# dmiruke/find_motion

Measured on NVIDIA B200. Metric: 1080p frames/sec (whole box), higher is better.
Workload: dtype u8+f64

## Files before the change

find_motion_b200/csrc/fm_common.cuh:

```cuda
#pragma once

#include <cuda.h>
#include <cuda_runtime.h>
#include <stdint.h>

#include <atomic>
#include <utility>

#include "../../include/fm_gpu.h"
#include "fm_device.cuh"

#define FM_MAX_K 1024
#define FM_TILE_PX 512
#define FM_TILE_WORDS 16
#define FM_TIMING_RING 16384
#define FM_MAX_DEVICES 64

struct StreamState {
    int has_bg;
    int counter;
    int decay;
    int cache_len;
};

// ... 18 lines not shown
    int *parent;
    int *area2;
    int *bbox;
};

struct fm_ctx {
    fm_config cfg;
    fm_info info;
    int S, Tmax, W, H, w, h, k, wpr;
    int N;
    int ntiles;
    int resize_mode;
    size_t frame_bytes;
    uint8_t *nv12_bgr;
    bool fused;
    bool wide_fused;
    bool umma;
    uint8_t *uband;
    uint8_t *uband_f;
    bool umma_direct;
    int umma_ra;
    uint8_t *gpad;
    int fx, fy;
    int maxc;
    int *coef;
    uint32_t *wtab;
    ResizeTab xtab, ytab;
    int *g4start, *g4n, *g4off;
    float4 *g4w;
    int g4max;
// ... 76 lines not shown
#define FM_LAUNCH_CHECK()                                                         \
    do {                                                                          \
        g_launches.fetch_add(1, std::memory_order_relaxed);                       \
        cudaError_t e_ = cudaGetLastError();                                      \
        if (e_ != cudaSuccess) {                                                  \
            fm_set_error("kernel launch failed: %s (%s:%d)", cudaGetErrorString(e_), \
                         __FILE__, __LINE__);                                     \
            return FM_ECUDA;                                                      \
        }                                                                         \
    } while (0)

inline uint32_t *fm_tflat(const fm_ctx *c) {
    return c->tflat + (size_t)c->slot * c->S * c->Tmax * c->ntiles * FM_TILE_WORDS;
}
inline int *fm_rawrange(const fm_ctx *c) { return c->rawrange + (size_t)c->slot * 6 * c->S * c->Tmax; }

template <typename... KArgs, typename... Args>
cudaError_t fm_launch_chained(void (*kernel)(KArgs...), dim3 grid, dim3 block, size_t smem, cudaStream_t st,
                              Args &&...args) {
    cudaLaunchAttribute at[1];
    at[0].id = cudaLaunchAttributeProgrammaticStreamSerialization;
    at[0].val.programmaticStreamSerializationAllowed = 1;
    cudaLaunchConfig_t cfg = {};
    cfg.gridDim = grid; cfg.blockDim = block; cfg.dynamicSmemBytes = smem; cfg.stream = st;
    cfg.attrs = at; cfg.numAttrs = 1;
    return cudaLaunchKernelEx(&cfg, kernel, std::forward<Args>(args)...);
}
__device__ __forceinline__ unsigned long long fm_globaltimer() {
    unsigned long long t;
    asm volatile("mov.u64 %0, %%globaltimer;" : "=l"(t));
// ... 15 lines not shown
int fm_frames_tmap(const fm_ctx *c, const uint8_t *frames, size_t sstride, size_t fstride, int T, int box_words, int box_rows,
                   CUtensorMap *out);

int fm_launch_frontend(fm_ctx *c, const uint8_t *frames, size_t sstride, size_t fstride, int T,
                       cudaStream_t st);
int fm_launch_temporal(fm_ctx *c, int T, cudaStream_t st);
int fm_launch_fused(fm_ctx *c, const uint8_t *frames, size_t sstride, size_t fstride, int T, cudaStream_t st);
int fm_ccl_configure(fm_ctx *c);
int fm_launch_morph_ccl(fm_ctx *c, int T, cudaStream_t st, fm_frame_stats *stats_out);
int fm_launch_masks(fm_ctx *c, int stream, int n_polys, const int *offs, const int *pts_scaled,
                    int npts, cudaStream_t st);
int fm_launch_bg_export(fm_ctx *c, int stream, double *dst_dev, cudaStream_t st);
int fm_launch_thresh_export(fm_ctx *c, int stream, int t, uint8_t *dst_dev, cudaStream_t st);
int fm_launch_mask_export(fm_ctx *c, int stream, uint8_t *dst_dev, cudaStream_t st);
bool fm_fused_supported(const fm_ctx *c);
size_t fm_wide_plane_bytes(const fm_ctx *c);
int fm_wide_init(fm_ctx *c, const int *taps);
bool fm_wide_fused_supported(const fm_ctx *c);
size_t fm_wide_bg_doubles(const fm_ctx *c);
int fm_launch_bg_export_wide(fm_ctx *c, int stream, double *dst_dev, cudaStream_t st);
int fm_launch_wide_blur(fm_ctx *c, const uint8_t *frames, size_t sstride, size_t fstride, int T, cudaStream_t st);
size_t fm_fused_bg_doubles(const fm_ctx *c);
int fm_launch_bg_export_fused(fm_ctx *c, int stream, double *dst_dev, cudaStream_t st);
int fm_launch_resize_bgr(int device, const uint8_t *src_dev, size_t sstride, size_t fstride, int S, int T, int W, int H,
                         int w, int h, int mode, int fx, int fy, const ResizeTab &xt, const ResizeTab &yt, const int *oidx,
                         uint8_t *dst_dev, size_t ostride, cudaStream_t st);
size_t fm_upscale_smem(int w);
int fm_launch_upscale(int device, const uint8_t *frames, size_t sstride, size_t fstride, int T, int F, int W, int H, int w,
                      int h, const int2 *xt, const int2 *yt, const int *nvalid, uint8_t *gray, uint8_t *bgr_out,
                      const int *oidx, size_t ostride, cudaStream_t st);
// ... 30 lines not shown
```

find_motion_b200/csrc/fm_host.cu:

```cuda
#include <ctype.h>
#include <math.h>
#include <stdarg.h>
#include <stdio.h>
#include <stdlib.h>
#include <string.h>

#include <algorithm>
#include <map>
#include <mutex>
#include <utility>
#include <vector>

#include <sched.h>
#include <unistd.h>

#include "fm_common.cuh"

std::atomic<unsigned long long> g_launches{0};
static thread_local char g_err[512] = "";

int fm_ensure_smem(const void *func, size_t bytes, int device) {
    static std::mutex mu;
    static std::map<std::pair<const void *, int>, size_t> done;
    std::lock_guard<std::mutex> lk(mu);
// ... 379 lines not shown
    FM_TRY(cudaMemset(c->errflag, 0, sizeof(int)));
    FM_TRY(cudaMemset(c->heavy, 0, F * sizeof(int)));
    int cap = c->w / 4 + 3;
    size_t per_frame = (size_t)c->h * cap * 28 + (size_t)c->h * 4 + 4;
    size_t budget = (size_t)8 << 30;
    int nb = (int)std::min<size_t>(F, std::max<size_t>(1, budget / per_frame));
    if ((rc = fm_ccl_alloc(&c->ccl, nb, c->h, cap))) return fail(rc);
    if ((rc = fm_ccl_configure(c))) return fail(rc);
    if ((cfg->flags & FM_FLAG_DEVICE_CLIPS) && (rc = fm_clips_alloc(c))) return fail(rc);
#ifdef FM_NV12_STAGED
    const bool nv12_staged = true;
#else
    const bool nv12_staged = !c->fused;
#endif
    if ((cfg->flags & FM_FLAG_NV12) && nv12_staged) ALLOC(c->nv12_bgr, F * c->W * c->H * 3);
    if (cfg->flags & FM_FLAG_OBJECT_PLANES) {
        const int ow = FM_OBJECT_WIDTH;
        c->obj_h = obj_h;
        if (ow < c->W) {
            const double sx = 1.0 / ((double)ow / W), sy = 1.0 / ((double)obj_h / H);
            const int isx = (int)nearbyint(sx), isy = (int)nearbyint(sy);
            if (fabs(sx - isx) < 2.220446049250313e-16 && fabs(sy - isy) < 2.220446049250313e-16) {
                c->obj_mode = 2; c->obj_fx = isx; c->obj_fy = isy;
            } else {
                c->obj_mode = 1;
                const HostTab xt = area_tab(c->W, ow), yt = area_tab(c->H, obj_h);
                if ((rc = upload_tab(&c->obj_xtab, xt)) || (rc = upload_tab(&c->obj_ytab, yt))) return fail(rc);
                if ((rc = fm_rows_plan_objects(c, xt.start.data(), xt.idx.data(), xt.wt.data(), yt.start.data(), yt.idx.data())))
                    return fail(rc);
            }
// ... 573 lines not shown
```

find_motion_b200/csrc/k_fused.cu:

```cuda
#include <cuda.h>

#include "fm_common.cuh"

#define FT_W 128
#ifndef FT_H
#define FT_H 32
#endif
#define FT_PX 16
#define FUSED_WARPS (FT_H / 4)
#define FG_WORDS 36
#define FG_ROWS (FT_H + 4)
#define FH_MB ((FG_ROWS + 15) / 16)
#define FH_ROWS (16 * FH_MB)
#ifndef FUSED_MIN_CTAS
#define FUSED_MIN_CTAS (1024 / (8 * FT_H))
#endif
#define FH_WORDS 68
#define FUSED_THREADS (8 * FT_H)
#define RAW_PITCH 432
#define RAW_BYTES (RAW_PITCH * FG_ROWS)
#define RAW_STAGE ((RAW_BYTES + 127) / 128 * 128)
#define NV_PITCH 160
#define NV_Y_BYTES (NV_PITCH * FG_ROWS)
#define NV_BYTES (NV_Y_BYTES + NV_PITCH * FG_ROWS / 2)

struct FusedParams {
    int T, w, h, wpr;
    const int *nvalid;
    int tilesX, tilesY;
    double *bg;
    const uint32_t *maskbits;
    uint32_t *tbits;
    size_t flatwords;
    const int *bg_in;
    int *bg_out;
    int *clear_ff;
    int *clear_zero;
    int n_ff, n_zero;
    unsigned long long *stamp;
    int b0, b1, b2, shift, rnd;
    int threshold;
    double alpha, beta;
    int qoff; uint32_t nthr2; double nC;
    uint8_t *gray_out, *blur_out;
    int *rawrange;
    uint4 bfr[32];
#ifdef FM_K1_PROF
    long long *prof;
#endif
};

enum { K1_WAIT, K1_GRAY, K1_BORDER, K1_HORIZ, K1_VERT, K1_TAIL, K1_NPROF };
#ifdef FM_K1_PROF
#define K1_PROF(slot)                                \
    do {                                             \
        if (tid == 0) {                              \
            const long long now_ = clock64();        \
            k1_prof[slot] += now_ - k1_prof_t;       \
            k1_prof_t = now_;                        \
        }                                            \
    } while (0)
#else
#define K1_PROF(slot) do {} while (0)
#endif

static void fused_bfr(FusedParams &p) {
    for (int lane = 0; lane < 32; lane++) {
// ... 76 lines not shown
            fm_temporal_px<SAFE, INIT>(sv, bg[idx], bits, p.threshold, p.qoff, p.nthr2, p.alpha, p.beta, p.nC);
        }
    }
    return __brev(bits) >> (32 - FT_PX);
}

__device__ __forceinline__ void rawrange_hit(const FusedParams &p, int s, int t, int y) {
    int *rr = p.rawrange + 2 * ((size_t)s * p.T + t);
    atomicMax(rr, min(y + 3, p.h - 1));
    atomicMax(rr + 1, p.h - 1 - y);
}

__device__ __forceinline__ void fused_exit(const FusedParams &p) {
    fm_stamp_end(p.stamp);
    fm_wait_predecessor();
    const int nthreads = gridDim.x * gridDim.y * gridDim.z * FUSED_THREADS;
    for (int i = ((blockIdx.z * gridDim.y + blockIdx.y) * gridDim.x + blockIdx.x) * FUSED_THREADS + threadIdx.x;
         i < p.n_ff + p.n_zero; i += nthreads) {
        if (i < p.n_ff) p.clear_ff[i] = -1;
        else p.clear_zero[i - p.n_ff] = 0;
    }
}

__device__ __forceinline__ uint32_t nv12_gray4(uint32_t y4, const FmChroma &c0, const FmChroma &c1) {
    return fm_nv12_gray(y4 & 0xFFu, c0) | (fm_nv12_gray((y4 >> 8) & 0xFFu, c0) << 8) |
           (fm_nv12_gray((y4 >> 16) & 0xFFu, c1) << 16) | (fm_nv12_gray(y4 >> 24, c1) << 24);
}

template <bool KEEP, bool SAFE, bool NV12>
__global__ void __launch_bounds__(FUSED_THREADS, FUSED_MIN_CTAS) k_fused(const __grid_constant__ CUtensorMap tmap, FusedParams p,
                                                                         const __grid_constant__ CUtensorMap tmap_uv) {
    extern __shared__ __align__(128) unsigned char fsm[];
    unsigned char *raw = fsm;
    uint32_t *sg = reinterpret_cast<uint32_t *>(fsm + 2 * RAW_STAGE);
    uint32_t *sh = sg + FH_ROWS * FG_WORDS;
    uint64_t *bars = reinterpret_cast<uint64_t *>(sh + FH_ROWS * FH_WORDS);
    const int tid = threadIdx.x, lane = tid & 31, warp = tid >> 5;
    const int s = blockIdx.z;
    const int tx = blockIdx.x, ty = blockIdx.y, tile = ty * p.tilesX + tx;
    const int x0 = tx * FT_W, y0 = ty * FT_H;
    const int w = p.w, h = p.h;
    const bool border = (x0 == 0) || (x0 + FT_W >= w) || (y0 == 0) || (y0 + FT_H >= h);
    fm_stamp_start(p.stamp);
    const bool has_bg = p.bg_in[s] != 0;
    const int Ts = min(p.T, __ldg(p.nvalid + s));
    if (tid == 0 && tx == 0 && ty == 0) p.bg_out[s] = has_bg || Ts > 0;
    if (Ts <= 0) {
        fused_exit(p);
        return;
    }

    const int trow = tid >> 3, xg = tid & 7;
    const int px = x0 + 8 * xg, py = y0 + trow;
    double2 *bgt = reinterpret_cast<double2 *>(p.bg) +
                   ((((size_t)s * p.tilesX * p.tilesY + tile) * FUSED_WARPS + warp) * (FT_PX / 2)) * 32 + lane;
    double bg[FT_PX];
    if (has_bg) {
#pragma unroll
        for (int i = 0; i < FT_PX / 2; i++) {
            double2 v = bgt[i * 32];
            bg[2 * i] = v.x;
            bg[2 * i + 1] = v.y;
        }
    }
    uint32_t M = 0;
    const bool okA = py < h && px < w, okB = py < h && px + 64 < w;
    const uint32_t vmask = (okA ? 1u : 0u) | (okB ? 2u : 0u);
    if (okA) M = (__ldg(p.maskbits + ((size_t)s * h + py) * p.wpr + (px >> 5)) >> (px & 31)) & 0xFFu;
    if (okB) M |= ((__ldg(p.maskbits + ((size_t)s * h + py) * p.wpr + ((px + 64) >> 5)) >> (px & 31)) & 0xFFu) << 8;
    const bool wmasked = __any_sync(0xffffffffu, M != 0);
    const int cx = (x0 * 3) / 4 - 4, cy = y0 - 2;
    if (tid == 0) {
        fm_mbar_init(&bars[0], 1);
        fm_mbar_init(&bars[1], 1);
        asm volatile("fence.mbarrier_init.release.cluster;" ::: "memory");
        asm volatile("fence.proxy.async.shared::cta;" ::: "memory");
    }
    __syncthreads();
    if (tid == 0) {
        if (NV12) {
            fm_mbar_expect_tx(&bars[0], NV_BYTES);
            fm_tma_load_4d(raw, &tmap, &bars[0], x0 / 4 - 4, y0 - 2, 0, s);
            fm_tma_load_4d(raw + NV_Y_BYTES, &tmap_uv, &bars[0], x0 / 4 - 4, y0 / 2 - 1, 0, s);
        } else {
            fm_mbar_expect_tx(&bars[0], RAW_BYTES);
            fm_tma_load_4d(raw, &tmap, &bars[0], cx, cy, 0, s);
        }
    }
    uint8_t *tb = reinterpret_cast<uint8_t *>(p.tbits + ((size_t)s * p.T) * p.flatwords + (size_t)py * p.wpr) + (px >> 3);
    uint32_t bfr[2][2];
    {
        const uint4 b = p.bfr[lane];
        bfr[0][0] = b.x; bfr[0][1] = b.y; bfr[1][0] = b.z; bfr[1][1] = b.w;
        asm volatile("" : "+r"(bfr[0][0]), "+r"(bfr[0][1]), "+r"(bfr[1][0]), "+r"(bfr[1][1]));
    }
    const int hwin = warp & 7;
    const uint32_t sg_lane = fm_smem_u32(sg) + ((lane & 7) + 8 * ((lane >> 3) & 1)) * (FG_WORDS * 4) + 16 * hwin + 16 * (lane >> 4);
    uint32_t *sh_lane = sh + (lane >> 2) * FH_WORDS + 8 * hwin + (lane & 3);
    const int rs_tid = 4 + 24 * tid;
    uint2 *const sgt = reinterpret_cast<uint2 *>(sg) + tid;
    const uint32_t bars_s = fm_smem_u32(bars);
    uint32_t hits = 0;
#ifdef FM_K1_PROF
    long long k1_prof[K1_NPROF] = {}, k1_prof_t = clock64();
#endif

    for (int t = 0; t < Ts; t++) {
        if (tid == 0 && t + 1 < Ts) {
            if (NV12) {
                unsigned char *dst = raw + ((t + 1) & 1) * RAW_STAGE;
                fm_mbar_expect_tx(&bars[(t + 1) & 1], NV_BYTES);
                fm_tma_load_4d(dst, &tmap, &bars[(t + 1) & 1], x0 / 4 - 4, y0 - 2, t + 1, s);
                fm_tma_load_4d(dst + NV_Y_BYTES, &tmap_uv, &bars[(t + 1) & 1], x0 / 4 - 4, y0 / 2 - 1, t + 1, s);
            } else {
                fm_mbar_expect_tx(&bars[(t + 1) & 1], RAW_BYTES);
                fm_tma_load_4d(raw + ((t + 1) & 1) * RAW_STAGE, &tmap, &bars[(t + 1) & 1], cx, cy, t + 1, s);
            }
        }
        fm_mbar_wait(bars_s + 8 * (t & 1), (t >> 1) & 1);
        K1_PROF(K1_WAIT);
        if (NV12) {
            constexpr int NU = (FG_ROWS / 2) * FG_WORDS, NFULL = NU / FUSED_THREADS;
            const unsigned char *st = raw + (t & 1) * RAW_STAGE;
#pragma unroll
            for (int i = 0; i <= NFULL; i++) {
                if (i < NFULL || tid < NU - NFULL * FUSED_THREADS) {
                    const int un = tid + i * FUSED_THREADS, k = un / FG_WORDS, u = un - k * FG_WORDS;
                    const unsigned char *yq = st + 2 * k * NV_PITCH + 12 + 4 * u;
                    const uint32_t l0 = *reinterpret_cast<const uint32_t *>(yq);
                    const uint32_t l1 = *reinterpret_cast<const uint32_t *>(yq + NV_PITCH);
                    const uint32_t cw = *reinterpret_cast<const uint32_t *>(st + NV_Y_BYTES + k * NV_PITCH + 12 + 4 * u);
                    const FmChroma c0 = fm_nv12_chroma(cw & 0xFFu, (cw >> 8) & 0xFFu);
                    const FmChroma c1 = fm_nv12_chroma((cw >> 16) & 0xFFu, cw >> 24);
                    sg[2 * k * FG_WORDS + u] = nv12_gray4(l0, c0, c1);
                    sg[(2 * k + 1) * FG_WORDS + u] = nv12_gray4(l1, c0, c1);
                }
            }
        } else {
            constexpr int NU = FG_ROWS * FG_WORDS / 2, NFULL = NU / FUSED_THREADS;
            const unsigned char *rs = raw + (t & 1) * RAW_STAGE + rs_tid;
#pragma unroll
            for (int i = 0; i <= NFULL; i++) {
                if (i < NFULL || tid < NU - NFULL * FUSED_THREADS) {
                    const unsigned char *q = rs + i * (24 * FUSED_THREADS);
                    const uint32_t a0 = *reinterpret_cast<const uint32_t *>(q), a5 = *reinterpret_cast<const uint32_t *>(q + 20);
                    const uint2 a12 = *reinterpret_cast<const uint2 *>(q + 4), a34 = *reinterpret_cast<const uint2 *>(q + 12);
                    const uint32_t g0 = fm_gray4(a0, a12.x, a12.y), g1 = fm_gray4(a34.x, a34.y, a5);
                    sgt[i * FUSED_THREADS] = make_uint2(g0, g1);
                }
            }
        }
        __syncthreads();
        K1_PROF(K1_GRAY);
        if (border) {
            unsigned char *sb = reinterpret_cast<unsigned char *>(sg);
            for (int ry = tid; ry < FG_ROWS; ry += FUSED_THREADS) {
                unsigned char *row = sb + ry * (FG_WORDS * 4) + 4;
                if (x0 == 0) { row[-1] = row[1]; row[-2] = row[2]; }
                if (x0 + FT_W >= w) { int e = w - x0; row[e] = row[e - 2]; row[e + 1] = row[e - 3]; }
            }
            __syncthreads();
            for (int i = tid; i < FG_WORDS; i += FUSED_THREADS) {
                if (y0 == 0) { sg[1 * FG_WORDS + i] = sg[3 * FG_WORDS + i]; sg[0 * FG_WORDS + i] = sg[4 * FG_WORDS + i]; }
                if (y0 + FT_H >= h) {
                    int e = h - y0 + 2;
                    sg[e * FG_WORDS + i] = sg[(e - 2) * FG_WORDS + i];
                    sg[(e + 1) * FG_WORDS + i] = sg[(e - 3) * FG_WORDS + i];
                }
            }
            __syncthreads();
        }
        K1_PROF(K1_BORDER);
        if (KEEP) {
            for (int u = tid; u < FT_H * (FT_W / 4); u += FUSED_THREADS) {
                int ry = u / (FT_W / 4), ux = u - ry * (FT_W / 4);
                int gy = y0 + ry, gx = x0 + 4 * ux;
                if (gy < h && gx < w)
                    *reinterpret_cast<uint32_t *>(p.gray_out + (((size_t)s * p.T + t) * h + gy) * w + gx) =
                        sg[(ry + 2) * FG_WORDS + ux + 1];
            }
        }
        {
            constexpr int MBS = FUSED_WARPS / 8;
            constexpr int NMB = (FH_MB + MBS - 1) / MBS;
            const int mb0 = warp >> 3;
            uint32_t a[NMB][4];
#pragma unroll
            for (int i = 0; i < NMB; i++)
                if (MBS == 1 || mb0 + i * MBS < FH_MB) fm_ldsm_x4(sg_lane + (mb0 + i * MBS) * (16 * FG_WORDS * 4), a[i]);
#pragma unroll
            for (int i = 0; i < NMB; i++) {
                if (MBS == 1 || mb0 + i * MBS < FH_MB) {
                    int d0[4], d1[4];
                    fm_imma0(d0, a[i][0], a[i][1], a[i][2], a[i][3], bfr[0][0], bfr[0][1], 0);
                    fm_imma0(d1, a[i][0], a[i][1], a[i][2], a[i][3], bfr[1][0], bfr[1][1], 0);
                    uint32_t *o = sh_lane + (mb0 + i * MBS) * (16 * FH_WORDS);
                    o[0] = __byte_perm(d0[0], d0[1], 0x5410);
                    o[4] = __byte_perm(d1[0], d1[1], 0x5410);
                    o[8 * FH_WORDS] = __byte_perm(d0[2], d0[3], 0x5410);
                    o[8 * FH_WORDS + 4] = __byte_perm(d1[2], d1[3], 0x5410);
                }
            }
        }
        __syncthreads();
        K1_PROF(K1_HORIZ);
        const uint32_t *sgw = sh + trow * FH_WORDS + 4 * xg;
        asm volatile("" : "+r"(M));
        uint8_t *bo = KEEP ? p.blur_out + (((size_t)s * p.T + t) * h + py) * w + px : nullptr;
        uint32_t bits;
        if (t == 0 && !has_bg) bits = fused_rows<KEEP, SAFE, true, true, false>(sgw, bg, M, p, bo, vmask);
        else if (wmasked) bits = p.shift == 8 ? fused_rows<KEEP, SAFE, false, true, true>(sgw, bg, M, p, bo, vmask)
                                              : fused_rows<KEEP, SAFE, false, true, false>(sgw, bg, M, p, bo, vmask);
        else if (p.shift == 8) bits = fused_rows<KEEP, SAFE, false, false, true>(sgw, bg, M, p, bo, vmask);
        else bits = fused_rows<KEEP, SAFE, false, false, false>(sgw, bg, M, p, bo, vmask);
        K1_PROF(K1_VERT);
        if (!okA) bits = 0;
        if (!okB) bits &= 0xFFu;
        if (okA) tb[0] = (uint8_t)bits;
        if (okB) tb[8] = (uint8_t)(bits >> 8);
        const bool any = __any_sync(0xffffffffu, bits != 0);
        if (Ts <= 32) hits |= (any ? 1u : 0u) << t;
        else if (any && lane == 0) rawrange_hit(p, s, t, y0 + 4 * warp);
        tb += 4 * p.flatwords;
        K1_PROF(K1_TAIL);
    }
#ifdef FM_K1_PROF
    if (tid == 0) {
        for (int i = 0; i < K1_NPROF; i++) atomicAdd((unsigned long long *)p.prof + i, (unsigned long long)k1_prof[i]);
        atomicAdd((unsigned long long *)p.prof + K1_NPROF, (unsigned long long)Ts);
    }
#endif
    if (Ts <= 32 && ((hits >> lane) & 1u)) rawrange_hit(p, s, lane, y0 + 4 * warp);
#pragma unroll
    for (int i = 0; i < FT_PX / 2; i++) bgt[i * 32] = make_double2(bg[2 * i], bg[2 * i + 1]);
    fused_exit(p);
}

__global__ void k_bg_export_fused(const double *__restrict__ bg, double *__restrict__ dst, int w, int h, int tilesX,
                                  int tilesY, int s) {
    int x = blockIdx.x * blockDim.x + threadIdx.x, y = blockIdx.y;
    if (x >= w) return;
    int tx = x / FT_W, ty = y / FT_H, tile = ty * tilesX + tx;
    int lx = x - tx * FT_W, ly = y - ty * FT_H;
    int tid = ly * 8 + ((lx & 63) >> 3);
    int warp = tid >> 5, lane = tid & 31;
    int idx = 8 * (lx >> 6) + (lx & 7);
    size_t base = ((((size_t)s * tilesX * tilesY + tile) * FUSED_WARPS + warp) * (FT_PX / 2)) * 32;
    dst[(size_t)y * w + x] = bg[(base + (size_t)(idx >> 1) * 32 + lane) * 2 + (idx & 1)];
}
// ... 11 lines not shown
#include <cstdio>
#include <cstring>

static long long *k1_prof_buffer() {
    static long long *buf = nullptr;
    if (!buf && cudaMallocManaged(&buf, (K1_NPROF + 1) * sizeof(long long)) == cudaSuccess)
        memset(buf, 0, (K1_NPROF + 1) * sizeof(long long));
    return buf;
}

extern "C" void fm_k1_prof_dump(void) {
    long long *b = k1_prof_buffer();
    if (!b) return;
    cudaDeviceSynchronize();
    const double n = b[K1_NPROF] ? (double)b[K1_NPROF] : 1.0;
    fprintf(stderr, "k1 phases (cycles per CTA-frame, thread 0, %lld CTA-frames): wait %.1f gray %.1f border %.1f "
            "horizontal %.1f vertical %.1f tail %.1f\n", b[K1_NPROF], b[K1_WAIT] / n, b[K1_GRAY] / n, b[K1_BORDER] / n,
            b[K1_HORIZ] / n, b[K1_VERT] / n, b[K1_TAIL] / n);
    memset(b, 0, (K1_NPROF + 1) * sizeof(long long));
}
#endif

#define FUSED_SMEM (2 * RAW_STAGE + FH_ROWS * FG_WORDS * 4 + FH_ROWS * FH_WORDS * 4 + 16)

static int nv12_plane_tmap(const fm_ctx *c, const uint8_t *plane, int rows, size_t sstride, size_t fstride, int T,
                           int box_rows, CUtensorMap *out) {
    PFN_encodeTiled enc = fm_tma_encoder();
    if (!enc) { fm_set_error("cuTensorMapEncodeTiled not available"); return FM_ECUDA; }
    const size_t dense = c->frame_bytes;
    cuuint64_t dims[4] = {(cuuint64_t)c->W / 4, (cuuint64_t)rows, (cuuint64_t)T, (cuuint64_t)c->S};
    cuuint64_t strides[3] = {(cuuint64_t)c->W, (cuuint64_t)(T > 1 ? fstride : dense),
                             (cuuint64_t)(c->S > 1 ? sstride : (T > 1 ? fstride * T : dense))};
    cuuint32_t box[4] = {NV_PITCH / 4, (cuuint32_t)box_rows, 1, 1};
    cuuint32_t estr[4] = {1, 1, 1, 1};
    CUresult r = enc(out, CU_TENSOR_MAP_DATA_TYPE_UINT32, 4, (void *)plane, dims, strides, box, estr, CU_TENSOR_MAP_INTERLEAVE_NONE,
                     CU_TENSOR_MAP_SWIZZLE_NONE, CU_TENSOR_MAP_L2_PROMOTION_L2_128B, CU_TENSOR_MAP_FLOAT_OOB_FILL_NONE);
    if (r != CUDA_SUCCESS) { fm_set_error("cuTensorMapEncodeTiled (NV12 plane) failed (%d)", (int)r); return FM_ECUDA; }
    return FM_OK;
}

int fm_launch_fused(fm_ctx *c, const uint8_t *frames, size_t sstride, size_t fstride, int T, cudaStream_t st) {
    CUtensorMap tmap, tmap_uv;
    const bool nv12 = c->nv12_bgr == nullptr && (c->cfg.flags & FM_FLAG_NV12);
    int rc;
    if (nv12) {
        if ((((uintptr_t)frames) | sstride | fstride) & 15) {
            fm_set_error("the fused NV12 front end needs 16-byte aligned frames and strides");
            return FM_EINVAL;
        }
        if ((rc = nv12_plane_tmap(c, frames, c->H, sstride, fstride, T, FG_ROWS, &tmap))) return rc;
        if ((rc = nv12_plane_tmap(c, frames + (size_t)c->W * c->H, c->H / 2, sstride, fstride, T, FG_ROWS / 2, &tmap_uv))) return rc;
    } else {
        if ((rc = fm_frames_tmap(c, frames, sstride, fstride, T, RAW_PITCH / 4, FG_ROWS, &tmap))) return rc;
        tmap_uv = tmap;
    }
    FusedParams p;
    p.T = T; p.nvalid = c->nvalid;
    p.w = c->w; p.h = c->h; p.wpr = c->wpr;
    p.tilesX = (c->w + FT_W - 1) / FT_W; p.tilesY = (c->h + FT_H - 1) / FT_H;
    p.bg = c->bg; p.maskbits = c->maskbits; p.tbits = fm_tflat(c);
    p.flatwords = (size_t)c->ntiles * FM_TILE_WORDS;
    p.bg_in = c->bg_valid + (size_t)c->slot * c->S;
    p.bg_out = c->bg_valid + (size_t)(c->slot ^ 1) * c->S;
    {
        const int Fmax = c->S * c->Tmax;
        p.clear_ff = c->rawrange + (c->slot ? 0 : 2 * Fmax);
        p.n_ff = 6 * Fmax;
        p.clear_zero = c->ncomp;
        p.n_zero = 2 * Fmax + 4;
    }
    int lg;
    if (c->k == 1) { p.b0 = 0; p.b1 = 0; p.b2 = 1; lg = 8; }
    else if (c->k == 3) { p.b0 = 0; p.b1 = 1; p.b2 = 2; lg = 6; }
    else { p.b0 = 1; p.b1 = 4; p.b2 = 6; lg = 4; }
    p.shift = 16 - 2 * lg;
    int r1 = p.shift ? (1 << (p.shift - 1)) : 0;
    p.rnd = r1 | (r1 << 16);
    p.threshold = c->cfg.threshold;
    p.alpha = c->cfg.avg; p.beta = 1.0 - p.alpha;
    p.qoff = (int)(0x4B400000u - (unsigned)p.threshold); p.nthr2 = ~(2u * (unsigned)p.threshold); p.nC = -(4503599627370496.0 * p.alpha);
    p.gray_out = c->gray; p.blur_out = c->blur;
    p.rawrange = fm_rawrange(c);
    p.stamp = c->stamp;
#ifdef FM_K1_PROF
    p.prof = k1_prof_buffer();
    if (!p.prof) return FM_ECUDA;
#endif
    const bool keep = (c->cfg.flags & FM_FLAG_KEEP_PLANES) != 0;
    const bool safe = p.alpha >= 0.0 && p.alpha <= 1.0 && p.threshold >= 0;
    fused_bfr(p);
    dim3 grid(p.tilesX, p.tilesY, c->S);
    typedef void (*FusedKernel)(const CUtensorMap, FusedParams, const CUtensorMap);
    const FusedKernel kerns[2][2][2] = {{{k_fused<false, false, false>, k_fused<false, false, true>},
                                         {k_fused<false, true, false>, k_fused<false, true, true>}},
                                        {{k_fused<true, false, false>, k_fused<true, false, true>},
                                         {k_fused<true, true, false>, k_fused<true, true, true>}}};
    const FusedKernel kern = kerns[keep][safe][nv12];
    if ((rc = fm_ensure_smem((const void *)kern, FUSED_SMEM, c->cfg.device))) return rc;
    if (c->nv12_bgr) kern<<<grid, FUSED_THREADS, FUSED_SMEM, st>>>(tmap, p, tmap_uv);
    else (void)fm_launch_chained(kern, grid, dim3(FUSED_THREADS), FUSED_SMEM, st, tmap, p, tmap_uv);
    FM_LAUNCH_CHECK();
    return FM_OK;
}

int fm_launch_bg_export_fused(fm_ctx *c, int stream, double *dst_dev, cudaStream_t st) {
    dim3 grid((c->w + 127) / 128, c->h);
    k_bg_export_fused<<<grid, 128, 0, st>>>(c->bg, dst_dev, c->w, c->h, (c->w + FT_W - 1) / FT_W,
                                            (c->h + FT_H - 1) / FT_H, stream);
    FM_LAUNCH_CHECK();
    return FM_OK;
}
```

Measured before the change: 376,900.

## Convert fused front-end kernel to persistent CTAs with atomic tile work queue

The fused gray/blur/background kernel is changed from one CTA per (tile, stream) into a persistent grid sized to the number of resident CTAs. Each CTA pulls tiles from a global atomic counter. The TMA load for the next tile's first frame is issued during the current tile's last frame, and L2 prefetches of the next frame and of the next tile's background block are added. Border handling is folded into the gray conversion through row reflection and byte permutes, replacing the separate border pass. The aim is to remove launch and tail imbalance and hide load latency across tile boundaries, at the cost of atomic contention, a per-slot queue counter that must be cleared, and more complex index logic.

```diff
diff --git a/find_motion_b200/csrc/fm_common.cuh b/find_motion_b200/csrc/fm_common.cuh
--- a/find_motion_b200/csrc/fm_common.cuh
+++ b/find_motion_b200/csrc/fm_common.cuh
@@ -56,6 +56,7 @@
     size_t frame_bytes;
     uint8_t *nv12_bgr;
     bool fused;
+    int fused_ctas;
     bool wide_fused;
     bool umma;
     uint8_t *uband;
@@ -162,6 +163,7 @@
     return c->tflat + (size_t)c->slot * c->S * c->Tmax * c->ntiles * FM_TILE_WORDS;
 }
 inline int *fm_rawrange(const fm_ctx *c) { return c->rawrange + (size_t)c->slot * 6 * c->S * c->Tmax; }
+inline int *fm_k1_queue(const fm_ctx *c) { return c->ncomp + 2 * (size_t)c->S * c->Tmax + 2; }
 
 template <typename... KArgs, typename... Args>
 cudaError_t fm_launch_chained(void (*kernel)(KArgs...), dim3 grid, dim3 block, size_t smem, cudaStream_t st,
@@ -207,6 +209,7 @@
 int fm_launch_thresh_export(fm_ctx *c, int stream, int t, uint8_t *dst_dev, cudaStream_t st);
 int fm_launch_mask_export(fm_ctx *c, int stream, uint8_t *dst_dev, cudaStream_t st);
 bool fm_fused_supported(const fm_ctx *c);
+int fm_fused_init(fm_ctx *c);
 size_t fm_wide_plane_bytes(const fm_ctx *c);
 int fm_wide_init(fm_ctx *c, const int *taps);
 bool fm_wide_fused_supported(const fm_ctx *c);
diff --git a/find_motion_b200/csrc/fm_host.cu b/find_motion_b200/csrc/fm_host.cu
--- a/find_motion_b200/csrc/fm_host.cu
+++ b/find_motion_b200/csrc/fm_host.cu
@@ -417,6 +417,7 @@
     const bool nv12_staged = !c->fused;
 #endif
     if ((cfg->flags & FM_FLAG_NV12) && nv12_staged) ALLOC(c->nv12_bgr, F * c->W * c->H * 3);
+    if (c->fused && (rc = fm_fused_init(c))) return fail(rc);
     if (cfg->flags & FM_FLAG_OBJECT_PLANES) {
         const int ow = FM_OBJECT_WIDTH;
         c->obj_h = obj_h;
diff --git a/find_motion_b200/csrc/k_fused.cu b/find_motion_b200/csrc/k_fused.cu
--- a/find_motion_b200/csrc/k_fused.cu
+++ b/find_motion_b200/csrc/k_fused.cu
@@ -1,4 +1,6 @@
 #include <cuda.h>
+
+#include <algorithm>
 
 #include "fm_common.cuh"
 
@@ -28,6 +30,9 @@
     int T, w, h, wpr;
     const int *nvalid;
     int tilesX, tilesY;
+    int tiles, items;
+    int *queue;
+    int *queue_clear;
     double *bg;
     const uint32_t *maskbits;
     uint32_t *tbits;
@@ -50,7 +55,7 @@
 #endif
 };
 
-enum { K1_WAIT, K1_GRAY, K1_BORDER, K1_HORIZ, K1_VERT, K1_TAIL, K1_NPROF };
+enum { K1_WAIT, K1_GRAY, K1_HORIZ, K1_VERT, K1_TAIL, K1_NPROF };
 #ifdef FM_K1_PROF
 #define K1_PROF(slot)                                \
     do {                                             \
@@ -157,11 +162,62 @@
 __device__ __forceinline__ void fused_exit(const FusedParams &p) {
     fm_stamp_end(p.stamp);
     fm_wait_predecessor();
-    const int nthreads = gridDim.x * gridDim.y * gridDim.z * FUSED_THREADS;
-    for (int i = ((blockIdx.z * gridDim.y + blockIdx.y) * gridDim.x + blockIdx.x) * FUSED_THREADS + threadIdx.x;
-         i < p.n_ff + p.n_zero; i += nthreads) {
+    const int nthreads = gridDim.x * FUSED_THREADS;
+    for (int i = blockIdx.x * FUSED_THREADS + threadIdx.x; i <= p.n_ff + p.n_zero; i += nthreads) {
         if (i < p.n_ff) p.clear_ff[i] = -1;
-        else p.clear_zero[i - p.n_ff] = 0;
+        else if (i < p.n_ff + p.n_zero) p.clear_zero[i - p.n_ff] = 0;
+        else *p.queue_clear = 0;
+    }
+}
+
+__device__ __forceinline__ int fused_src_row(int r, int y0, int h) {
+    if (y0 == 0 && r < 2) return 4 - r;
+    const int e = h - y0 + 2;
+    return (r == e || r == e + 1) ? 2 * e - 2 - r : r;
+}
+
+__device__ __forceinline__ void fused_item(const FusedParams &p, int it, int &s, int &tile, int &x0, int &y0) {
+    s = it / p.tiles;
+    tile = it - s * p.tiles;
+    const int ty = tile / p.tilesX;
+    x0 = (tile - ty * p.tilesX) * FT_W;
+    y0 = ty * FT_H;
+}
+
+__device__ __forceinline__ int fused_take(const FusedParams &p, int &ts) {
+    for (;;) {
+        const int it = atomicAdd(p.queue, 1);
+        if (it >= p.items) return p.items;
+        const int s = it / p.tiles;
+        ts = min(p.T, __ldg(p.nvalid + s));
+        if (it == s * p.tiles) p.bg_out[s] = p.bg_in[s] != 0 || ts > 0;
+        if (ts > 0) return it;
+    }
+}
+
+__device__ __forceinline__ void fm_tma_prefetch_4d(const CUtensorMap *map, int c0, int c1, int c2, int c3) {
+    asm volatile("cp.async.bulk.prefetch.tensor.4d.L2.global.tile [%0, {%1, %2, %3, %4}];"
+                 ::"l"(map), "r"(c0), "r"(c1), "r"(c2), "r"(c3) : "memory");
+}
+__device__ __forceinline__ void fm_bulk_prefetch(const void *src, uint32_t bytes) {
+    asm volatile("cp.async.bulk.prefetch.L2.global [%0], %1;" ::"l"(src), "r"(bytes) : "memory");
+}
+
+template <bool NV12>
+__device__ __forceinline__ void fused_load(unsigned char *dst, uint64_t *bar, const CUtensorMap *tmap, const CUtensorMap *tmap_uv,
+                                           int x0, int y0, int t, int s, bool next) {
+    if (NV12) {
+        fm_mbar_expect_tx(bar, NV_BYTES);
+        fm_tma_load_4d(dst, tmap, bar, x0 / 4 - 4, y0 - 2, t, s);
+        fm_tma_load_4d(dst + NV_Y_BYTES, tmap_uv, bar, x0 / 4 - 4, y0 / 2 - 1, t, s);
+        if (next) {
+            fm_tma_prefetch_4d(tmap, x0 / 4 - 4, y0 - 2, t + 1, s);
+            fm_tma_prefetch_4d(tmap_uv, x0 / 4 - 4, y0 / 2 - 1, t + 1, s);
+        }
+    } else {
+        fm_mbar_expect_tx(bar, RAW_BYTES);
+        fm_tma_load_4d(dst, tmap, bar, (x0 * 3) / 4 - 4, y0 - 2, t, s);
+        if (next) fm_tma_prefetch_4d(tmap, (x0 * 3) / 4 - 4, y0 - 2, t + 1, s);
     }
 }
 
@@ -178,59 +234,11 @@
     uint32_t *sg = reinterpret_cast<uint32_t *>(fsm + 2 * RAW_STAGE);
     uint32_t *sh = sg + FH_ROWS * FG_WORDS;
     uint64_t *bars = reinterpret_cast<uint64_t *>(sh + FH_ROWS * FH_WORDS);
+    __shared__ int next_item[2];
     const int tid = threadIdx.x, lane = tid & 31, warp = tid >> 5;
-    const int s = blockIdx.z;
-    const int tx = blockIdx.x, ty = blockIdx.y, tile = ty * p.tilesX + tx;
-    const int x0 = tx * FT_W, y0 = ty * FT_H;
     const int w = p.w, h = p.h;
-    const bool border = (x0 == 0) || (x0 + FT_W >= w) || (y0 == 0) || (y0 + FT_H >= h);
     fm_stamp_start(p.stamp);
-    const bool has_bg = p.bg_in[s] != 0;
-    const int Ts = min(p.T, __ldg(p.nvalid + s));
-    if (tid == 0 && tx == 0 && ty == 0) p.bg_out[s] = has_bg || Ts > 0;
-    if (Ts <= 0) {
-        fused_exit(p);
-        return;
-    }
-
     const int trow = tid >> 3, xg = tid & 7;
-    const int px = x0 + 8 * xg, py = y0 + trow;
-    double2 *bgt = reinterpret_cast<double2 *>(p.bg) +
-                   ((((size_t)s * p.tilesX * p.tilesY + tile) * FUSED_WARPS + warp) * (FT_PX / 2)) * 32 + lane;
-    double bg[FT_PX];
-    if (has_bg) {
-#pragma unroll
-        for (int i = 0; i < FT_PX / 2; i++) {
-            double2 v = bgt[i * 32];
-            bg[2 * i] = v.x;
-            bg[2 * i + 1] = v.y;
-        }
-    }
-    uint32_t M = 0;
-    const bool okA = py < h && px < w, okB = py < h && px + 64 < w;
-    const uint32_t vmask = (okA ? 1u : 0u) | (okB ? 2u : 0u);
-    if (okA) M = (__ldg(p.maskbits + ((size_t)s * h + py) * p.wpr + (px >> 5)) >> (px & 31)) & 0xFFu;
-    if (okB) M |= ((__ldg(p.maskbits + ((size_t)s * h + py) * p.wpr + ((px + 64) >> 5)) >> (px & 31)) & 0xFFu) << 8;
-    const bool wmasked = __any_sync(0xffffffffu, M != 0);
-    const int cx = (x0 * 3) / 4 - 4, cy = y0 - 2;
-    if (tid == 0) {
-        fm_mbar_init(&bars[0], 1);
-        fm_mbar_init(&bars[1], 1);
-        asm volatile("fence.mbarrier_init.release.cluster;" ::: "memory");
-        asm volatile("fence.proxy.async.shared::cta;" ::: "memory");
-    }
-    __syncthreads();
-    if (tid == 0) {
-        if (NV12) {
-            fm_mbar_expect_tx(&bars[0], NV_BYTES);
-            fm_tma_load_4d(raw, &tmap, &bars[0], x0 / 4 - 4, y0 - 2, 0, s);
-            fm_tma_load_4d(raw + NV_Y_BYTES, &tmap_uv, &bars[0], x0 / 4 - 4, y0 / 2 - 1, 0, s);
-        } else {
-            fm_mbar_expect_tx(&bars[0], RAW_BYTES);
-            fm_tma_load_4d(raw, &tmap, &bars[0], cx, cy, 0, s);
-        }
-    }
-    uint8_t *tb = reinterpret_cast<uint8_t *>(p.tbits + ((size_t)s * p.T) * p.flatwords + (size_t)py * p.wpr) + (px >> 3);
     uint32_t bfr[2][2];
     {
         const uint4 b = p.bfr[lane];
@@ -243,139 +251,210 @@
     const int rs_tid = 4 + 24 * tid;
     uint2 *const sgt = reinterpret_cast<uint2 *>(sg) + tid;
     const uint32_t bars_s = fm_smem_u32(bars);
-    uint32_t hits = 0;
+    if (tid == 0) {
+        fm_mbar_init(&bars[0], 1);
+        fm_mbar_init(&bars[1], 1);
+        asm volatile("fence.mbarrier_init.release.cluster;" ::: "memory");
+        asm volatile("fence.proxy.async.shared::cta;" ::: "memory");
+        int ts = 0;
+        const int it = fused_take(p, ts);
+        next_item[0] = it;
+        if (it < p.items) {
+            int s, tile, x0, y0;
+            fused_item(p, it, s, tile, x0, y0);
+            fused_load<NV12>(raw, &bars[0], &tmap, &tmap_uv, x0, y0, 0, s, ts > 1);
+        }
+    }
+    __syncthreads();
+    uint32_t f = 0;
 #ifdef FM_K1_PROF
     long long k1_prof[K1_NPROF] = {}, k1_prof_t = clock64();
 #endif
-
-    for (int t = 0; t < Ts; t++) {
-        if (tid == 0 && t + 1 < Ts) {
-            if (NV12) {
-                unsigned char *dst = raw + ((t + 1) & 1) * RAW_STAGE;
-                fm_mbar_expect_tx(&bars[(t + 1) & 1], NV_BYTES);
-                fm_tma_load_4d(dst, &tmap, &bars[(t + 1) & 1], x0 / 4 - 4, y0 - 2, t + 1, s);
-                fm_tma_load_4d(dst + NV_Y_BYTES, &tmap_uv, &bars[(t + 1) & 1], x0 / 4 - 4, y0 / 2 - 1, t + 1, s);
-            } else {
-                fm_mbar_expect_tx(&bars[(t + 1) & 1], RAW_BYTES);
-                fm_tma_load_4d(raw + ((t + 1) & 1) * RAW_STAGE, &tmap, &bars[(t + 1) & 1], cx, cy, t + 1, s);
+    for (int n = 0;; n++) {
+        const int it = next_item[n & 1];
+        if (it >= p.items) break;
+        int s, tile, x0, y0;
+        fused_item(p, it, s, tile, x0, y0);
+        const bool border = (x0 == 0) || (x0 + FT_W >= w) || (y0 == 0) || (y0 + FT_H + 1 >= h);
+        const bool has_bg = p.bg_in[s] != 0;
+        const int Ts = min(p.T, __ldg(p.nvalid + s));
+        const int px = x0 + 8 * xg, py = y0 + trow;
+        double2 *bgt = reinterpret_cast<double2 *>(p.bg) + (((size_t)it * FUSED_WARPS + warp) * (FT_PX / 2)) * 32 + lane;
+        double bg[FT_PX];
+        if (has_bg) {
+#pragma unroll
+            for (int i = 0; i < FT_PX / 2; i++) {
+                double2 v = bgt[i * 32];
+                bg[2 * i] = v.x;
+                bg[2 * i + 1] = v.y;
             }
         }
-        fm_mbar_wait(bars_s + 8 * (t & 1), (t >> 1) & 1);
-        K1_PROF(K1_WAIT);
-        if (NV12) {
-            constexpr int NU = (FG_ROWS / 2) * FG_WORDS, NFULL = NU / FUSED_THREADS;
-            const unsigned char *st = raw + (t & 1) * RAW_STAGE;
-#pragma unroll
-            for (int i = 0; i <= NFULL; i++) {
-                if (i < NFULL || tid < NU - NFULL * FUSED_THREADS) {
-                    const int un = tid + i * FUSED_THREADS, k = un / FG_WORDS, u = un - k * FG_WORDS;
-                    const unsigned char *yq = st + 2 * k * NV_PITCH + 12 + 4 * u;
-                    const uint32_t l0 = *reinterpret_cast<const uint32_t *>(yq);
-                    const uint32_t l1 = *reinterpret_cast<const uint32_t *>(yq + NV_PITCH);
-                    const uint32_t cw = *reinterpret_cast<const uint32_t *>(st + NV_Y_BYTES + k * NV_PITCH + 12 + 4 * u);
-                    const FmChroma c0 = fm_nv12_chroma(cw & 0xFFu, (cw >> 8) & 0xFFu);
-                    const FmChroma c1 = fm_nv12_chroma((cw >> 16) & 0xFFu, cw >> 24);
-                    sg[2 * k * FG_WORDS + u] = nv12_gray4(l0, c0, c1);
-                    sg[(2 * k + 1) * FG_WORDS + u] = nv12_gray4(l1, c0, c1);
+        uint32_t M = 0;
+        const bool okA = py < h && px < w, okB = py < h && px + 64 < w;
+        const uint32_t vmask = (okA ? 1u : 0u) | (okB ? 2u : 0u);
+        if (okA) M = (__ldg(p.maskbits + ((size_t)s * h + py) * p.wpr + (px >> 5)) >> (px & 31)) & 0xFFu;
+        if (okB) M |= ((__ldg(p.maskbits + ((size_t)s * h + py) * p.wpr + ((px + 64) >> 5)) >> (px & 31)) & 0xFFu) << 8;
+        const bool wmasked = __any_sync(0xffffffffu, M != 0);
+        uint8_t *tb = reinterpret_cast<uint8_t *>(p.tbits + ((size_t)s * p.T) * p.flatwords + (size_t)py * p.wpr) + (px >> 3);
+        uint32_t hits = 0;
+
+        for (int t = 0; t < Ts; t++, f++) {
+            if (tid == 0) {
+                unsigned char *dst = raw + ((f + 1) & 1) * RAW_STAGE;
+                uint64_t *bar = &bars[(f + 1) & 1];
+                if (t + 1 < Ts) {
+                    fused_load<NV12>(dst, bar, &tmap, &tmap_uv, x0, y0, t + 1, s, t + 2 < Ts);
+                } else {
+                    int ts = 0;
+                    const int nx = fused_take(p, ts);
+                    next_item[(n + 1) & 1] = nx;
+                    if (nx < p.items) {
+                        int ns, ntile, nx0, ny0;
+                        fused_item(p, nx, ns, ntile, nx0, ny0);
+                        fused_load<NV12>(dst, bar, &tmap, &tmap_uv, nx0, ny0, 0, ns, ts > 1);
+                        if (p.bg_in[ns] != 0)
+                            fm_bulk_prefetch(reinterpret_cast<const double2 *>(p.bg) + (size_t)nx * FUSED_WARPS * (FT_PX / 2) * 32,
+                                             FUSED_WARPS * (FT_PX / 2) * 32 * sizeof(double2));
+                    }
                 }
             }
-        } else {
-            constexpr int NU = FG_ROWS * FG_WORDS / 2, NFULL = NU / FUSED_THREADS;
-            const unsigned char *rs = raw + (t & 1) * RAW_STAGE + rs_tid;
-#pragma unroll
-            for (int i = 0; i <= NFULL; i++) {
-                if (i < NFULL || tid < NU - NFULL * FUSED_THREADS) {
-                    const unsigned char *q = rs + i * (24 * FUSED_THREADS);
-                    const uint32_t a0 = *reinterpret_cast<const uint32_t *>(q), a5 = *reinterpret_cast<const uint32_t *>(q + 20);
-                    const uint2 a12 = *reinterpret_cast<const uint2 *>(q + 4), a34 = *reinterpret_cast<const uint2 *>(q + 12);
-                    const uint32_t g0 = fm_gray4(a0, a12.x, a12.y), g1 = fm_gray4(a34.x, a34.y, a5);
-                    sgt[i * FUSED_THREADS] = make_uint2(g0, g1);
+            fm_mbar_wait(bars_s + 8 * (f & 1), (f >> 1) & 1);
+            K1_PROF(K1_WAIT);
+            if (NV12) {
+                constexpr int NU = (FG_ROWS / 2) * FG_WORDS, NFULL = NU / FUSED_THREADS;
+                const unsigned char *st = raw + (f & 1) * RAW_STAGE;
+#pragma unroll
+                for (int i = 0; i <= NFULL; i++) {
+                    if (i < NFULL || tid < NU - NFULL * FUSED_THREADS) {
+                        const int un = tid + i * FUSED_THREADS, k = un / FG_WORDS, u = un - k * FG_WORDS;
+                        if (!border) {
+                            const unsigned char *yq = st + 2 * k * NV_PITCH + 12 + 4 * u;
+                            const uint32_t l0 = *reinterpret_cast<const uint32_t *>(yq);
+                            const uint32_t l1 = *reinterpret_cast<const uint32_t *>(yq + NV_PITCH);
+                            const uint32_t cw = *reinterpret_cast<const uint32_t *>(st + NV_Y_BYTES + k * NV_PITCH + 12 + 4 * u);
+                            const FmChroma c0 = fm_nv12_chroma(cw & 0xFFu, (cw >> 8) & 0xFFu);
+                            const FmChroma c1 = fm_nv12_chroma((cw >> 16) & 0xFFu, cw >> 24);
+                            sg[2 * k * FG_WORDS + u] = nv12_gray4(l0, c0, c1);
+                            sg[(2 * k + 1) * FG_WORDS + u] = nv12_gray4(l1, c0, c1);
+                        } else {
+                            const int r0 = fused_src_row(2 * k, y0, h), r1 = fused_src_row(2 * k + 1, y0, h);
+                            int us = u;
+                            uint32_t sel = 0x3210;
+                            if (x0 == 0 && u == 0) { us = 1; sel = 0x1200; }
+                            if (x0 + FT_W >= w && u == (w - x0) / 4 + 1) { us = u - 1; sel = 0x3212; }
+                            const unsigned char *yq = st + 12 + 4 * us, *cq = st + NV_Y_BYTES + 12 + 4 * us;
+                            const uint32_t l0 = *reinterpret_cast<const uint32_t *>(yq + r0 * NV_PITCH);
+                            const uint32_t l1 = *reinterpret_cast<const uint32_t *>(yq + r1 * NV_PITCH);
+                            uint32_t cw = *reinterpret_cast<const uint32_t *>(cq + (r0 >> 1) * NV_PITCH);
+                            FmChroma c0 = fm_nv12_chroma(cw & 0xFFu, (cw >> 8) & 0xFFu);
+                            FmChroma c1 = fm_nv12_chroma((cw >> 16) & 0xFFu, cw >> 24);
+                            sg[2 * k * FG_WORDS + u] = __byte_perm(nv12_gray4(l0, c0, c1), 0, sel);
+                            if ((r1 >> 1) != (r0 >> 1)) {
+                                cw = *reinterpret_cast<const uint32_t *>(cq + (r1 >> 1) * NV_PITCH);
+                                c0 = fm_nv12_chroma(cw & 0xFFu, (cw >> 8) & 0xFFu);
+                                c1 = fm_nv12_chroma((cw >> 16) & 0xFFu, cw >> 24);
+                            }
+                            sg[(2 * k + 1) * FG_WORDS + u] = __byte_perm(nv12_gray4(l1, c0, c1), 0, sel);
+                        }
+                    }
                 }
-            }
-        }
-        __syncthreads();
-        K1_PROF(K1_GRAY);
-        if (border) {
-            unsigned char *sb = reinterpret_cast<unsigned char *>(sg);
-            for (int ry = tid; ry < FG_ROWS; ry += FUSED_THREADS) {
-                unsigned char *row = sb + ry * (FG_WORDS * 4) + 4;
-                if (x0 == 0) { row[-1] = row[1]; row[-2] = row[2]; }
-                if (x0 + FT_W >= w) { int e = w - x0; row[e] = row[e - 2]; row[e + 1] = row[e - 3]; }
-            }
-            __syncthreads();
-            for (int i = tid; i < FG_WORDS; i += FUSED_THREADS) {
-                if (y0 == 0) { sg[1 * FG_WORDS + i] = sg[3 * FG_WORDS + i]; sg[0 * FG_WORDS + i] = sg[4 * FG_WORDS + i]; }
-                if (y0 + FT_H >= h) {
-                    int e = h - y0 + 2;
-                    sg[e * FG_WORDS + i] = sg[(e - 2) * FG_WORDS + i];
-                    sg[(e + 1) * FG_WORDS + i] = sg[(e - 3) * FG_WORDS + i];
+            } else {
+                constexpr int NU = FG_ROWS * FG_WORDS / 2, NFULL = NU / FUSED_THREADS;
+                if (border) {
+                    const unsigned char *stg = raw + (f & 1) * RAW_STAGE + 4;
+                    const int ecu = x0 + FT_W >= w ? (w - x0) / 8 : -1;
+#pragma unroll
+                    for (int i = 0; i <= NFULL; i++) {
+                        if (i < NFULL || tid < NU - NFULL * FUSED_THREADS) {
+                            const int un = tid + i * FUSED_THREADS, r = un / (FG_WORDS / 2), c = un - r * (FG_WORDS / 2);
+                            const unsigned char *q = stg + fused_src_row(r, y0, h) * RAW_PITCH + 24 * c;
+                            const uint32_t a0 = *reinterpret_cast<const uint32_t *>(q), a5 = *reinterpret_cast<const uint32_t *>(q + 20);
+                            const uint2 a12 = *reinterpret_cast<const uint2 *>(q + 4), a34 = *reinterpret_cast<const uint2 *>(q + 12);
+                            uint32_t g0 = fm_gray4(a0, a12.x, a12.y), g1 = fm_gray4(a34.x, a34.y, a5);
+                            if (x0 == 0 && c == 0) g0 = __byte_perm(g0, g1, 0x5610);
+                            if (c == ecu) g1 = __byte_perm(g1, g0, 0x3256);
+                            sgt[i * FUSED_THREADS] = make_uint2(g0, g1);
+                        }
+                    }
+                } else {
+                    const unsigned char *rs = raw + (f & 1) * RAW_STAGE + rs_tid;
+#pragma unroll
+                    for (int i = 0; i <= NFULL; i++) {
+                        if (i < NFULL || tid < NU - NFULL * FUSED_THREADS) {
+                            const unsigned char *q = rs + i * (24 * FUSED_THREADS);
+                            const uint32_t a0 = *reinterpret_cast<const uint32_t *>(q), a5 = *reinterpret_cast<const uint32_t *>(q + 20);
+                            const uint2 a12 = *reinterpret_cast<const uint2 *>(q + 4), a34 = *reinterpret_cast<const uint2 *>(q + 12);
+                            const uint32_t g0 = fm_gray4(a0, a12.x, a12.y), g1 = fm_gray4(a34.x, a34.y, a5);
+                            sgt[i * FUSED_THREADS] = make_uint2(g0, g1);
+                        }
+                    }
                 }
             }
             __syncthreads();
-        }
-        K1_PROF(K1_BORDER);
-        if (KEEP) {
-            for (int u = tid; u < FT_H * (FT_W / 4); u += FUSED_THREADS) {
-                int ry = u / (FT_W / 4), ux = u - ry * (FT_W / 4);
-                int gy = y0 + ry, gx = x0 + 4 * ux;
-                if (gy < h && gx < w)
-                    *reinterpret_cast<uint32_t *>(p.gray_out + (((size_t)s * p.T + t) * h + gy) * w + gx) =
-                        sg[(ry + 2) * FG_WORDS + ux + 1];
-            }
-        }
-        {
-            constexpr int MBS = FUSED_WARPS / 8;
-            constexpr int NMB = (FH_MB + MBS - 1) / MBS;
-            const int mb0 = warp >> 3;
-            uint32_t a[NMB][4];
-#pragma unroll
-            for (int i = 0; i < NMB; i++)
-                if (MBS == 1 || mb0 + i * MBS < FH_MB) fm_ldsm_x4(sg_lane + (mb0 + i * MBS) * (16 * FG_WORDS * 4), a[i]);
-#pragma unroll
-            for (int i = 0; i < NMB; i++) {
-                if (MBS == 1 || mb0 + i * MBS < FH_MB) {
-                    int d0[4], d1[4];
-                    fm_imma0(d0, a[i][0], a[i][1], a[i][2], a[i][3], bfr[0][0], bfr[0][1], 0);
-                    fm_imma0(d1, a[i][0], a[i][1], a[i][2], a[i][3], bfr[1][0], bfr[1][1], 0);
-                    uint32_t *o = sh_lane + (mb0 + i * MBS) * (16 * FH_WORDS);
-                    o[0] = __byte_perm(d0[0], d0[1], 0x5410);
-                    o[4] = __byte_perm(d1[0], d1[1], 0x5410);
-                    o[8 * FH_WORDS] = __byte_perm(d0[2], d0[3], 0x5410);
-                    o[8 * FH_WORDS + 4] = __byte_perm(d1[2], d1[3], 0x5410);
+            K1_PROF(K1_GRAY);
+            if (KEEP) {
+                for (int u = tid; u < FT_H * (FT_W / 4); u += FUSED_THREADS) {
+                    int ry = u / (FT_W / 4), ux = u - ry * (FT_W / 4);
+                    int gy = y0 + ry, gx = x0 + 4 * ux;
+                    if (gy < h && gx < w)
+                        *reinterpret_cast<uint32_t *>(p.gray_out + (((size_t)s * p.T + t) * h + gy) * w + gx) =
+                            sg[(ry + 2) * FG_WORDS + ux + 1];
                 }
             }
-        }
-        __syncthreads();
-        K1_PROF(K1_HORIZ);
-        const uint32_t *sgw = sh + trow * FH_WORDS + 4 * xg;
-        asm volatile("" : "+r"(M));
-        uint8_t *bo = KEEP ? p.blur_out + (((size_t)s * p.T + t) * h + py) * w + px : nullptr;
-        uint32_t bits;
-        if (t == 0 && !has_bg) bits = fused_rows<KEEP, SAFE, true, true, false>(sgw, bg, M, p, bo, vmask);
-        else if (wmasked) bits = p.shift == 8 ? fused_rows<KEEP, SAFE, false, true, true>(sgw, bg, M, p, bo, vmask)
-                                              : fused_rows<KEEP, SAFE, false, true, false>(sgw, bg, M, p, bo, vmask);
-        else if (p.shift == 8) bits = fused_rows<KEEP, SAFE, false, false, true>(sgw, bg, M, p, bo, vmask);
-        else bits = fused_rows<KEEP, SAFE, false, false, false>(sgw, bg, M, p, bo, vmask);
-        K1_PROF(K1_VERT);
-        if (!okA) bits = 0;
-        if (!okB) bits &= 0xFFu;
-        if (okA) tb[0] = (uint8_t)bits;
-        if (okB) tb[8] = (uint8_t)(bits >> 8);
-        const bool any = __any_sync(0xffffffffu, bits != 0);
-        if (Ts <= 32) hits |= (any ? 1u : 0u) << t;
-        else if (any && lane == 0) rawrange_hit(p, s, t, y0 + 4 * warp);
-        tb += 4 * p.flatwords;
-        K1_PROF(K1_TAIL);
+            {
+                constexpr int MBS = FUSED_WARPS / 8;
+                constexpr int NMB = (FH_MB + MBS - 1) / MBS;
+                const int mb0 = warp >> 3;
+                uint32_t a[NMB][4];
+#pragma unroll
+                for (int i = 0; i < NMB; i++)
+                    if (MBS == 1 || mb0 + i * MBS < FH_MB) fm_ldsm_x4(sg_lane + (mb0 + i * MBS) * (16 * FG_WORDS * 4), a[i]);
+#pragma unroll
+                for (int i = 0; i < NMB; i++) {
+                    if (MBS == 1 || mb0 + i * MBS < FH_MB) {
+                        int d0[4], d1[4];
+                        fm_imma0(d0, a[i][0], a[i][1], a[i][2], a[i][3], bfr[0][0], bfr[0][1], 0);
+                        fm_imma0(d1, a[i][0], a[i][1], a[i][2], a[i][3], bfr[1][0], bfr[1][1], 0);
+                        uint32_t *o = sh_lane + (mb0 + i * MBS) * (16 * FH_WORDS);
+                        o[0] = __byte_perm(d0[0], d0[1], 0x5410);
+                        o[4] = __byte_perm(d1[0], d1[1], 0x5410);
+                        o[8 * FH_WORDS] = __byte_perm(d0[2], d0[3], 0x5410);
+                        o[8 * FH_WORDS + 4] = __byte_perm(d1[2], d1[3], 0x5410);
+                    }
+                }
+            }
+            __syncthreads();
+            K1_PROF(K1_HORIZ);
+            const uint32_t *sgw = sh + trow * FH_WORDS + 4 * xg;
+            asm volatile("" : "+r"(M));
+            uint8_t *bo = KEEP ? p.blur_out + (((size_t)s * p.T + t) * h + py) * w + px : nullptr;
+            uint32_t bits;
+            if (t == 0 && !has_bg) bits = fused_rows<KEEP, SAFE, true, true, false>(sgw, bg, M, p, bo, vmask);
+            else if (wmasked) bits = p.shift == 8 ? fused_rows<KEEP, SAFE, false, true, true>(sgw, bg, M, p, bo, vmask)
+                                                  : fused_rows<KEEP, SAFE, false, true, false>(sgw, bg, M, p, bo, vmask);
+            else if (p.shift == 8) bits = fused_rows<KEEP, SAFE, false, false, true>(sgw, bg, M, p, bo, vmask);
+            else bits = fused_rows<KEEP, SAFE, false, false, false>(sgw, bg, M, p, bo, vmask);
+            K1_PROF(K1_VERT);
+            if (!okA) bits = 0;
+            if (!okB) bits &= 0xFFu;
+            if (okA) tb[0] = (uint8_t)bits;
+            if (okB) tb[8] = (uint8_t)(bits >> 8);
+            const bool any = __any_sync(0xffffffffu, bits != 0);
+            if (Ts <= 32) hits |= (any ? 1u : 0u) << t;
+            else if (any && lane == 0) rawrange_hit(p, s, t, y0 + 4 * warp);
+            tb += 4 * p.flatwords;
+            K1_PROF(K1_TAIL);
+        }
+        if (Ts <= 32 && ((hits >> lane) & 1u)) rawrange_hit(p, s, lane, y0 + 4 * warp);
+#pragma unroll
+        for (int i = 0; i < FT_PX / 2; i++) bgt[i * 32] = make_double2(bg[2 * i], bg[2 * i + 1]);
     }
 #ifdef FM_K1_PROF
     if (tid == 0) {
         for (int i = 0; i < K1_NPROF; i++) atomicAdd((unsigned long long *)p.prof + i, (unsigned long long)k1_prof[i]);
-        atomicAdd((unsigned long long *)p.prof + K1_NPROF, (unsigned long long)Ts);
-    }
-#endif
-    if (Ts <= 32 && ((hits >> lane) & 1u)) rawrange_hit(p, s, lane, y0 + 4 * warp);
-#pragma unroll
-    for (int i = 0; i < FT_PX / 2; i++) bgt[i * 32] = make_double2(bg[2 * i], bg[2 * i + 1]);
+        atomicAdd((unsigned long long *)p.prof + K1_NPROF, (unsigned long long)f);
+    }
+#endif
     fused_exit(p);
 }
 
@@ -417,8 +496,8 @@
     if (!b) return;
     cudaDeviceSynchronize();
     const double n = b[K1_NPROF] ? (double)b[K1_NPROF] : 1.0;
-    fprintf(stderr, "k1 phases (cycles per CTA-frame, thread 0, %lld CTA-frames): wait %.1f gray %.1f border %.1f "
-            "horizontal %.1f vertical %.1f tail %.1f\n", b[K1_NPROF], b[K1_WAIT] / n, b[K1_GRAY] / n, b[K1_BORDER] / n,
+    fprintf(stderr, "k1 phases (cycles per CTA-frame, thread 0, %lld CTA-frames): wait %.1f gray %.1f "
+            "horizontal %.1f vertical %.1f tail %.1f\n", b[K1_NPROF], b[K1_WAIT] / n, b[K1_GRAY] / n,
             b[K1_HORIZ] / n, b[K1_VERT] / n, b[K1_TAIL] / n);
     memset(b, 0, (K1_NPROF + 1) * sizeof(long long));
 }
@@ -442,9 +521,34 @@
     return FM_OK;
 }
 
+typedef void (*FusedKernel)(const CUtensorMap, FusedParams, const CUtensorMap);
+
+static bool fused_nv12(const fm_ctx *c) { return c->nv12_bgr == nullptr && (c->cfg.flags & FM_FLAG_NV12); }
+
+static FusedKernel fused_kernel(const fm_ctx *c) {
+    const bool keep = (c->cfg.flags & FM_FLAG_KEEP_PLANES) != 0;
+    const bool safe = c->cfg.avg >= 0.0 && c->cfg.avg <= 1.0 && c->cfg.threshold >= 0;
+    const FusedKernel kerns[2][2][2] = {{{k_fused<false, false, false>, k_fused<false, false, true>},
+                                         {k_fused<false, true, false>, k_fused<false, true, true>}},
+                                        {{k_fused<true, false, false>, k_fused<true, false, true>},
+                                         {k_fused<true, true, false>, k_fused<true, true, true>}}};
+    return kerns[keep][safe][fused_nv12(c)];
+}
+
+int fm_fused_init(fm_ctx *c) {
+    const FusedKernel kern = fused_kernel(c);
+    int rc, per_sm = 0, sms = 0;
+    if ((rc = fm_ensure_smem((const void *)kern, FUSED_SMEM, c->cfg.device))) return rc;
+    FM_CUDA(cudaOccupancyMaxActiveBlocksPerMultiprocessor(&per_sm, kern, FUSED_THREADS, FUSED_SMEM));
+    FM_CUDA(cudaDeviceGetAttribute(&sms, cudaDevAttrMultiProcessorCount, c->cfg.device));
+    if (per_sm < 1) { fm_set_error("k_fused cannot be resident on device %d", c->cfg.device); return FM_ECUDA; }
+    c->fused_ctas = per_sm * sms;
+    return FM_OK;
+}
+
 int fm_launch_fused(fm_ctx *c, const uint8_t *frames, size_t sstride, size_t fstride, int T, cudaStream_t st) {
     CUtensorMap tmap, tmap_uv;
-    const bool nv12 = c->nv12_bgr == nullptr && (c->cfg.flags & FM_FLAG_NV12);
+    const bool nv12 = fused_nv12(c);
     int rc;
     if (nv12) {
         if ((((uintptr_t)frames) | sstride | fstride) & 15) {
@@ -461,6 +565,7 @@
     p.T = T; p.nvalid = c->nvalid;
     p.w = c->w; p.h = c->h; p.wpr = c->wpr;
     p.tilesX = (c->w + FT_W - 1) / FT_W; p.tilesY = (c->h + FT_H - 1) / FT_H;
+    p.tiles = p.tilesX * p.tilesY; p.items = c->S * p.tiles;
     p.bg = c->bg; p.maskbits = c->maskbits; p.tbits = fm_tflat(c);
     p.flatwords = (size_t)c->ntiles * FM_TILE_WORDS;
     p.bg_in = c->bg_valid + (size_t)c->slot * c->S;
@@ -470,7 +575,9 @@
         p.clear_ff = c->rawrange + (c->slot ? 0 : 2 * Fmax);
         p.n_ff = 6 * Fmax;
         p.clear_zero = c->ncomp;
-        p.n_zero = 2 * Fmax + 4;
+        p.n_zero = 2 * Fmax + 2;
+        p.queue = fm_k1_queue(c) + c->slot;
+        p.queue_clear = fm_k1_queue(c) + (c->slot ^ 1);
     }
     int lg;
     if (c->k == 1) { p.b0 = 0; p.b1 = 0; p.b2 = 1; lg = 8; }
@@ -489,17 +596,9 @@
     p.prof = k1_prof_buffer();
     if (!p.prof) return FM_ECUDA;
 #endif
-    const bool keep = (c->cfg.flags & FM_FLAG_KEEP_PLANES) != 0;
-    const bool safe = p.alpha >= 0.0 && p.alpha <= 1.0 && p.threshold >= 0;
     fused_bfr(p);
-    dim3 grid(p.tilesX, p.tilesY, c->S);
-    typedef void (*FusedKernel)(const CUtensorMap, FusedParams, const CUtensorMap);
-    const FusedKernel kerns[2][2][2] = {{{k_fused<false, false, false>, k_fused<false, false, true>},
-                                         {k_fused<false, true, false>, k_fused<false, true, true>}},
-                                        {{k_fused<true, false, false>, k_fused<true, false, true>},
-                                         {k_fused<true, true, false>, k_fused<true, true, true>}}};
-    const FusedKernel kern = kerns[keep][safe][nv12];
-    if ((rc = fm_ensure_smem((const void *)kern, FUSED_SMEM, c->cfg.device))) return rc;
+    const dim3 grid(std::min(p.items, c->fused_ctas));
+    const FusedKernel kern = fused_kernel(c);
     if (c->nv12_bgr) kern<<<grid, FUSED_THREADS, FUSED_SMEM, st>>>(tmap, p, tmap_uv);
     else (void)fm_launch_chained(kern, grid, dim3(FUSED_THREADS), FUSED_SMEM, st, tmap, p, tmap_uv);
     FM_LAUNCH_CHECK();
```

Result: slower. 366,300, median of 6 (-2.8%).
